# noveens/reviews4rec

Measured on AMD Instinct MI355X. Metric: train ratings/sec, higher is better.
Workload: dtype f32

## Files before the change

include/r4r.h:

```cpp
#ifndef R4R_H
#define R4R_H

#include <stddef.h>
#include <stdint.h>

#ifdef __cplusplus
extern "C" {
#endif

#define R4R_OK 0
#define R4R_ERR_ARG (-1)
#define R4R_ERR_LAUNCH (-2)
#define R4R_ERR_WORKSPACE (-3)

int r4r_version(void);
const char *r4r_last_error(void);

size_t r4r_textcnn_ws_bytes(int64_t N, int T, int E, int F, int64_t V);
int r4r_textcnn_fwd(const float *table, int64_t V, const int64_t *idx,
                    const float *conv_w, const float *conv_b,
                    float *pooled, int32_t *argmax,
                    void *ws, size_t ws_bytes,
                    int64_t N, int T, int E, int F, void *stream);

// ... 64 lines not shown
                       int64_t N, int R, int L, void *stream);

int r4r_mse_fwd_bwd(const float *out, const float *y, float *se, float *g_out,
                    int64_t N, float denom, void *stream);

int r4r_sqdist_mean_fwd(const float *a, const float *b, float *out, int64_t N, int L, void *stream);
int r4r_sqdist_mean_bwd(const float *a, const float *b, const float *g_out, float *g_a, float *g_b,
                        int64_t N, int L, void *stream);

int r4r_adam_chunk_elems(void);
int r4r_adam_multi(int ntensor, const uint64_t *p, const uint64_t *g, const uint64_t *m, const uint64_t *v,
                   const int64_t *numel, float lr, double beta1, double beta2, float eps,
                   float weight_decay, int64_t step, const int64_t *step_dev, void *stream);
int r4r_adam_gathered(float *p, const float *gathered, int world, float *g_sum, float *m, float *v,
                      int64_t numel, float lr, double beta1, double beta2, float eps,
                      float weight_decay, int64_t step, void *stream);
int r4r_adam_gathered_guarded(float *p, const float *gathered, int world, float *g_sum, float *m, float *v,
                              int64_t numel, float lr, double beta1, double beta2, float eps,
                              float weight_decay, int64_t step, const uint32_t *abort_word, void *stream);

int r4r_peer_segment_create(int64_t bytes, void **ptr, uint8_t *handle);
int r4r_peer_segment_open(const uint8_t *handle, void **ptr);
int r4r_peer_segment_close(void *ptr);
int r4r_peer_segment_destroy(void *ptr);
int r4r_peer_push(const float *src, int64_t numel, const uint64_t *peer_dst, const uint64_t *peer_flags,
                  uint32_t *arrive, int rank, int world, uint32_t epoch, const uint32_t *wait_flags,
                  uint32_t *timed_out, double timeout_s, void *stream);
int r4r_peer_wait(const uint32_t *flags, int world, uint32_t epoch, uint32_t *timed_out, double timeout_s, void *stream);


#define R4R_CONV_AUTO 0
#define R4R_CONV_DIRECT 1
#define R4R_CONV_PROJECT 2
int r4r_deepconn_nparam(void);
int r4r_deepconn_layout(int E, int L, int64_t *offsets, int64_t *sizes, int64_t *total);
size_t r4r_deepconn_ws_bytes(int64_t B, int T, int E, int L, int64_t V);
size_t r4r_deepconn_ws_mult_offset(int64_t B, int T, int E, int L, int64_t V);
size_t r4r_deepconn_ws_count_offset(int64_t B, int T, int E, int L, int64_t V, int tower, int buffer);
size_t r4r_deepconn_ws_partials_offset(int64_t B, int T, int E, int L, int64_t V, int tower, int which);
size_t r4r_deepconn_ws_plan_offset(int64_t B, int T, int E, int L, int64_t V, int tower, int buffer, int which);
size_t r4r_deepconn_ws_state_offset(int64_t B, int T, int E, int L, int64_t V, int tower, int buffer, int which);
int r4r_deepconn_step(const float *table, int64_t V, const int64_t *user_idx, const int64_t *item_idx,
                      const float *y, float *flat_p, float *flat_g,
                      float *pred, float *se, float *sse_accum,
                      void *ws, size_t ws_bytes,
                      int64_t B, int T, int E, int L,
                      float dropout_p, int training, uint64_t seed, uint64_t offset,
                      float inv_denom, int conv_algo, int token_buffer, int tokens_ready,
                      const int64_t *next_user_idx, const int64_t *next_item_idx,
                      float *flat_m, float *flat_v, float lr, double beta1, double beta2, float eps,
                      float weight_decay, int64_t adam_step, void *stream);
int r4r_deepconn_tail_fold(int on);
int r4r_deepconn_tail(int64_t B, int E, int L);
int r4r_deepconn_tokens(const int64_t *user_idx, const int64_t *item_idx, void *ws, size_t ws_bytes,
                        int64_t B, int T, int E, int L, int64_t V, int conv_algo, int token_buffer,
                        int discard, void *stream);

#define R4R_TIMING_TEXTCNN_FWD 0
#define R4R_TIMING_TEXTCNN_WGRAD 1
#define R4R_TIMING_ADAM 2
#define R4R_TIMING_PROJ_GEMM 3
#define R4R_TIMING_PROJ_GATHER 4
#define R4R_TIMING_SLOTS 8
int r4r_timing_enable(int slot_mask);
int r4r_timing_read(int slot, double *total_ms, int64_t *count, int reset);

size_t r4r_mf_ws_bytes(int64_t B, int D, int64_t n_users, int64_t n_items);
size_t r4r_mf_ws_persist_bytes(int64_t B, int D, int64_t n_users, int64_t n_items);
size_t r4r_mf_ws_mult_offset(int64_t B, int D, int64_t n_users, int64_t n_items);
size_t r4r_mf_ws_grad_offset(int64_t B, int D, int64_t n_users, int64_t n_items, int which);
int r4r_mf_step(const int64_t *uid, const int64_t *iid, const float *y,
                const uint64_t *p, const uint64_t *m, const uint64_t *v,
                int64_t n_users, int64_t n_items, int D,
                float *pred, float *se, float *sse_accum, void *ws, size_t ws_bytes, int64_t B,
                float dropout_p, int training, uint64_t seed, uint64_t offset, float inv_denom,
                int sweep_period, int64_t sweep_base, int sweep_all,
                float lr, double beta1, double beta2, float eps, float weight_decay, int64_t adam_step,
                void *stream);

int r4r_mf_rows_flush(const uint64_t *p, const uint64_t *m, const uint64_t *v,
                      int64_t n_users, int64_t n_items, int D, void *ws, size_t ws_bytes, int64_t B,
                      int sweep_period, int64_t sweep_base,
                      float lr, double beta1, double beta2, float eps, float weight_decay, int64_t adam_step,
                      void *stream);
size_t r4r_mf_ws_flag_offset(int64_t B, int D, int64_t n_users, int64_t n_items);

int r4r_sse_accumulate(const float *se, int64_t n, float *accum, void *stream);

size_t r4r_mf_dp_block_bytes(int64_t B_pad, int D);
int r4r_mf_grad(const int64_t *uid, const int64_t *iid, const float *y, const uint64_t *p,
                const uint64_t *m, const uint64_t *v,
                int64_t n_users, int64_t n_items, int D, float *pred, float *se, void *block, float *mult,
                int64_t B, int64_t B_pad, float dropout_p, int training, uint64_t seed, uint64_t offset,
                float inv_denom, void *ws, int sweep_period, int64_t sweep_base,
                float lr, double beta1, double beta2, float eps, float weight_decay, int64_t adam_step,
                void *stream);
int r4r_mf_apply(const void *blocks, int world, int64_t B_pad, const uint64_t *p, const uint64_t *m,
                 const uint64_t *v, int64_t n_users, int64_t n_items, int D, void *ws, size_t ws_bytes,
                 int sweep_period, int64_t sweep_base, int sweep_all,
                 const float *se, int64_t se_n, float *sse_accum,
                 float lr, double beta1, double beta2, float eps, float weight_decay, int64_t adam_step,
                 void *stream);
int r4r_mf_grad_push(const int64_t *uid, const int64_t *iid, const float *y, const uint64_t *p,
                     const uint64_t *m, const uint64_t *v,
                     int64_t n_users, int64_t n_items, int D, float *pred, float *se, float *mult,
                     int64_t B, int64_t B_pad, float dropout_p, int training, uint64_t seed, uint64_t offset,
// ... 380 lines not shown
```

reviews4rec_amd/csrc/engine.hip:

```cpp
#include <stdlib.h>

#include "trace_device.h"
#include "textcnn.h"
#include "wgrad_device.h"
#include "tokens_device.h"
#include "adam_device.h"

namespace r4r {

constexpr int F_CONV = 100;
constexpr int FM_K = 8;
constexpr int MAX_L = 128;

enum { P_UCW = 0, P_UCB, P_UFW, P_UFB, P_ICW, P_ICB, P_IFW, P_IFB, P_FMV, P_FMLW, P_FMLB, P_GB, P_COUNT };

struct Layout {
    int64_t off[P_COUNT], size[P_COUNT], total;
};

static Layout make_layout(int E, int L) {
    Layout lay;
    const int64_t sz[P_COUNT] = {(int64_t)F_CONV * 3 * E, F_CONV, (int64_t)L * F_CONV, L,
                                 (int64_t)F_CONV * 3 * E, F_CONV, (int64_t)L * F_CONV, L,
                                 (int64_t)2 * L * FM_K, 2 * L, 1, 1};
    int64_t o = 0;
    for (int i = 0; i < P_COUNT; ++i) {
        lay.off[i] = o;
        lay.size[i] = sz[i];
        o += (sz[i] + 31) & ~(int64_t)31;
    }
    lay.total = o;
    return lay;
}

struct HeadArgs {
    const float *pmax[2]; const int *parg[2];
    const float *fc_w[2]; const float *fc_b[2];
    const float *V, *lin_w, *lin_b, *gbias;
    const float *y;
    float *pooled[2]; int *argmax[2];
    float *g_pooled[2];
    float *mult;
    float *x, *s, *g, *gz;
    float *pred, *se;
    int64_t B;
    int L, tiles, training, want_grad;
    float p_drop, inv_denom;
    uint64_t seed, offset;
    PlanArgs plan;
    int *plan_spent[2];
    TokenArgs marks;
    int mark_wgs;
};


constexpr int HEAD_MAX_TILES = 8;

#define SEL2(arr, s) ((s) ? (arr)[1] : (arr)[0])
HEAD_TRACE_DEFINE(r4r_debug_dc_head_trace)
template <int ML>
__global__ __launch_bounds__(256) void deepconn_head_wg_kernel(HeadArgs a) {
    if ((int64_t)blockIdx.x >= a.B) {
        const int fb = (int)blockIdx.x - (int)a.B, flag_wgs = (2 * a.plan.units + 3) / 4;
        if (fb < flag_wgs) {
            segment_flags_wave(a.plan, fb * 4 + (int)(threadIdx.x >> 6));
        } else {
            const HeadArgs &A = kernel_args<HeadArgs>();
            token_mark_block(A.marks, fb - flag_wgs, A.mark_wgs, 256);
        }
        return;
    }
    HEAD_STAMP(0)
    constexpr int N2 = 2 * ML, PARTS = 256 / N2;
    __shared__ float sw[2][ML][F_CONV + 1];
    __shared__ float sfb[N2], slw[N2], sz[N2];
    __shared__ float sV[N2][FM_K];
    __shared__ float sp[2][F_CONV + 4];
    __shared__ float red[N2][PARTS + 1];
    const int tid = threadIdx.x, lane = tid & 63, w = tid >> 6;
    const int64_t b = blockIdx.x;
    const int L = a.L, n = 2 * L;
    const float lin_b0 = a.lin_b[0], gbias0 = a.gbias[0], yb = a.y ? a.y[b] : 0.f;

    constexpr int FQ = F_CONV / 4;
    typedef float hq4 __attribute__((ext_vector_type(4)));
    constexpr int WREGS = (2 * ML * FQ + 255) / 256;
    hq4 wreg[WREGS];
    const int wtot = 2 * L * FQ;
#pragma unroll
    for (int k = 0; k < WREGS; ++k) {
        const int i = min(tid + 256 * k, wtot - 1);
        const int t = i >= L * FQ;
        wreg[k] = *reinterpret_cast<const hq4 *>(SEL2(a.fc_w, t) + 4 * (i - t * L * FQ));
    }
    const int tn = min(tid, n - 1);
    const float fbreg = SEL2(a.fc_b, tn >= L)[tn - (tn >= L ? L : 0)];
    const float lwreg = a.lin_w[tn];
    constexpr int VREGS = (N2 * FM_K + 255) / 256;
    float vreg[VREGS];
#pragma unroll
    for (int k = 0; k < VREGS; ++k) vreg[k] = a.V[min(tid + 256 * k, n * FM_K - 1)];
    if (b == 0 && tid < 2 && SEL2(a.plan_spent, tid)) SEL2(a.plan_spent, tid)[0] = 0;

    {
        const int t = w >> 1, f = lane + 64 * (w & 1), fc = min(f, F_CONV - 1);
        float best = -INFINITY;
        int bp = -1;
        if (a.tiles <= HEAD_MAX_TILES) {
            float v[HEAD_MAX_TILES];
            int pp[HEAD_MAX_TILES];
#pragma unroll
            for (int k = 0; k < HEAD_MAX_TILES; ++k) {
                const size_t o = ((size_t)b * a.tiles + min(k, a.tiles - 1)) * NP + fc;
                v[k] = SEL2(a.pmax, t)[o];
                pp[k] = SEL2(a.parg, t)[o];
            }
#pragma unroll
            for (int k = 0; k < HEAD_MAX_TILES; ++k)
                if (v[k] > best) { best = v[k]; bp = pp[k]; }
        } else {
            for (int k0 = 0; k0 < a.tiles; k0 += HEAD_MAX_TILES) {
                float v[HEAD_MAX_TILES];
                int pp[HEAD_MAX_TILES];
#pragma unroll
                for (int k = 0; k < HEAD_MAX_TILES; ++k) {
                    const bool in = k0 + k < a.tiles;
                    const size_t o = ((size_t)b * a.tiles + (in ? k0 + k : 0)) * NP + fc;
                    v[k] = in ? SEL2(a.pmax, t)[o] : -INFINITY;
                    pp[k] = SEL2(a.parg, t)[o];
                }
#pragma unroll
                for (int k = 0; k < HEAD_MAX_TILES; ++k)
                    if (v[k] > best) { best = v[k]; bp = pp[k]; }
            }
        }
        if (!(best > 0.f)) { best = 0.f; bp = -1; }
        if (f < F_CONV) {
            sp[t][f] = best;
            SEL2(a.pooled, t)[b * F_CONV + f] = best;
            SEL2(a.argmax, t)[b * F_CONV + f] = bp;
        }
    }
    HEAD_STAMP(1)
#pragma unroll
    for (int k = 0; k < WREGS; ++k) {
        const int i = tid + 256 * k;
        if (i < wtot) {
            const int t = i >= L * FQ, r = i - t * L * FQ, l = r / FQ, f0 = 4 * (r - l * FQ);
#pragma unroll
            for (int c = 0; c < 4; ++c) sw[t][l][f0 + c] = wreg[k][c];
        }
    }
    if (tid < n) { sfb[tid] = fbreg; slw[tid] = lwreg; }
#pragma unroll
    for (int k = 0; k < VREGS; ++k) {
        const int i = tid + 256 * k;
        if (i < n * FM_K) sV[i / FM_K][i % FM_K] = vreg[k];
    }
    __syncthreads();
    HEAD_STAMP(2)

    {
        const int o = tid / PARTS, part = tid - o * PARTS;
        if (o < n) {
            const int t = o / L, l = o - t * L;
            float acc = 0.f;
            for (int f = part; f < F_CONV; f += PARTS) acc = fmaf(sp[t][f], sw[t][l][f], acc);
            red[o][part] = acc;
        }
    }
    __syncthreads();
    const bool has_y = a.y != nullptr, want = has_y && a.want_grad;
    if (w == 0) {
        constexpr int NI = (N2 + 63) / 64;
        float xi[NI], mult[NI], lw[NI], gacc[NI];
#pragma unroll
        for (int u = 0; u < NI; ++u) {
            const int i = lane + 64 * u;
            xi[u] = 0.f; mult[u] = 1.f; gacc[u] = 0.f;
            lw[u] = (i < n) ? slw[i] : 0.f;
            if (i < n) {
                float acc = 0.f;
#pragma unroll
                for (int q = 0; q < PARTS; ++q) acc += red[i][q];
                xi[u] = acc + sfb[i];
            }
            if (a.training && a.p_drop > 0.f && i < n) {
                const uint32_t r = philox_first_word(a.offset + (uint64_t)(b * n + i), a.seed);
                const float uu = (float)(r >> 8) * (1.0f / 16777216.0f);
                mult[u] = (uu >= a.p_drop) ? 1.f / (1.f - a.p_drop) : 0.f;
            }
            xi[u] *= mult[u];
        }
        float inter = 0.f;
        float sk_keep[FM_K];
#pragma unroll
        for (int k = 0; k < FM_K; ++k) {
            float pv = 0.f, pv2 = 0.f, vv[NI];
#pragma unroll
            for (int u = 0; u < NI; ++u) {
                const int i = lane + 64 * u;
                vv[u] = (i < n) ? sV[i][k] : 0.f;
                pv += xi[u] * vv[u];
                pv2 += xi[u] * xi[u] * vv[u] * vv[u];
            }
            const float sk = wave_sum(pv);
            const float s2 = wave_sum(pv2);
            inter += sk * sk - s2;
#pragma unroll
            for (int u = 0; u < NI; ++u) gacc[u] += sk * vv[u] - xi[u] * vv[u] * vv[u];
            sk_keep[k] = sk;
        }
        float pl = 0.f;
#pragma unroll
        for (int u = 0; u < NI; ++u) pl += xi[u] * lw[u];
        const float lin = wave_sum(pl);
        const float pred = (0.5f * inter + lin + lin_b0) + gbias0;
        if (lane == 0) a.pred[b] = pred;
        if (has_y) {
            const float d = pred - yb;
            if (lane == 0) a.se[b] = d * d;
            if (want) {
                const float g = 2.f * d * a.inv_denom;
#pragma unroll
                for (int u = 0; u < NI; ++u) {
                    const int i = lane + 64 * u;
                    const float gx = g * (gacc[u] + lw[u]);
                    const float gz = gx * mult[u];
                    if (i < n) {
                        sz[i] = gz;
                        a.x[b * n + i] = xi[u];
                        a.gz[b * n + i] = gz;
                        a.mult[b * n + i] = mult[u];
                    }
                }
                if (lane < FM_K) {
                    float sv = 0.f;
#pragma unroll
                    for (int k = 0; k < FM_K; ++k) if (lane == k) sv = sk_keep[k];
                    a.s[b * FM_K + lane] = sv;
                }
                if (lane == 0) a.g[b] = g;
            }
        }
    }
    if (!want) return;
    __syncthreads();
    HEAD_STAMP(3)
    if (tid < 2 * F_CONV) {
        const int t = tid >= F_CONV, f = tid - t * F_CONV;
        float acc = 0.f;
        for (int l = 0; l < L; ++l) acc = fmaf(sz[t * L + l], sw[t][l][f], acc);
        SEL2(a.g_pooled, t)[b * F_CONV + f] = acc;
    }
    HEAD_STAMP(4)
}

struct HeadGradArgs {
    const float *pooled[2];
    const float *x, *s, *g, *gz;
    const float *V;
    const float *se;
    float *g_fc_w[2], *g_fc_b[2], *g_V, *g_lin_w, *g_lin_b, *g_gb;
    float *sse_accum;
    int64_t B;
    int L;
};

constexpr int HG_ROWS = 16, HG_COLS = 16;
template <bool STEP = false>
__device__ __forceinline__ void head_grad_block(const HeadGradArgs &a, int blk, const FlatAdam *opt = nullptr) {
    __shared__ float red[HG_ROWS][HG_COLS];
    const int ox = threadIdx.x & (HG_COLS - 1), rg = threadIdx.x / HG_COLS;
    const int L = a.L, n = 2 * L;
    const int n_fcw = L * F_CONV;
    const int seg[9] = {n_fcw, L, n_fcw, L, n * FM_K, n, 1, 1, 1};
    int o = blk * HG_COLS + ox;
    int which = -1, local = 0, acc_o = o;
#pragma unroll
    for (int k = 0; k < 9; ++k) {
        if (which < 0) {
            if (acc_o < seg[k]) { which = k; local = acc_o; }
            else acc_o -= seg[k];
        }
    }
    float P = 0.f, M = 0.f, V = 0.f;
    int po = 0;
    bool stepping = false;
    if constexpr (STEP) {
        if (opt->on && rg == 0 && which >= 0 && which < 8) {
            const float *dst = which == 0 ? a.g_fc_w[0] + local : (which == 1 ? a.g_fc_b[0] + local : (which == 2 ? a.g_fc_w[1] + local :
                  (which == 3 ? a.g_fc_b[1] + local : (which == 4 ? a.g_V + local : (which == 5 ? a.g_lin_w + local :
                  (which == 6 ? a.g_lin_b : a.g_gb))))));
            po = (int)(dst - opt->g);
            stepping = true;
        }
    }
    float s = 0.f;
    if (which >= 0) {
// ... 50 lines not shown
        }
        if constexpr (STEP) {
            if (stepping) {
                adam_elem(P, t, M, V, opt->s);
                opt->p[po] = P; opt->m[po] = M; opt->v[po] = V;
            }
        }
    }
}

BWD_TRACE_DEFINE(r4r_debug_dc_bwd_trace)
struct DcBackwardArgs {
    WgradArgs w;
    HeadGradArgs h;
    int hg_blocks;
    TokenArgs nx;
    PlanArgs plan;
};
__global__ __launch_bounds__(WG_THREADS, 8) void deepconn_backward_kernel(DcBackwardArgs) {
    const DcBackwardArgs &A = kernel_args<DcBackwardArgs>();
    const WgradArgs &w = A.w;
    const HeadGradArgs &h = A.h;
    const TokenArgs &nx = A.nx;
    const PlanArgs &plan = A.plan;
    const int hg_blocks = A.hg_blocks;
    BWD_STAMP(0, wall_clock64())
    BWD_STAMP(2, (unsigned long long)blockIdx.z + 1)
    if (blockIdx.z == 1 || blockIdx.z == 2) {
        wgrad_block(w, blockIdx.x, blockIdx.y, blockIdx.z - 1);
    } else if (blockIdx.z == 0) {
        for (int blk = blockIdx.y * gridDim.x + blockIdx.x; blk < hg_blocks; blk += gridDim.x * gridDim.y) {
            head_grad_block(h, blk);
            __syncthreads();
        }
    } else {
        const int np = plan.units > 0 ? 2 : 0, blk = blockIdx.y * gridDim.x + blockIdx.x;
        if (blk < np) segment_plan_block<WG_THREADS>(plan, blk);
        else token_mark_block(nx, blk - np, gridDim.x * gridDim.y - np, WG_THREADS);
    }
#ifdef R4R_TRACE
    __syncthreads();
#endif
    BWD_STAMP(1, wall_clock64())
}

struct DcFoldArgs {
    WgradArgs w;
    FlatAdam opt;
    HeadGradArgs h;
    int hg_blocks;
    TokenArgs nx;
    PlanArgs plan;
    int comp_blocks;
};
static_assert(WG_THREADS % 64 == 0, "the 256-thread roles of the fold launch are whole waves: the others end before any barrier");
template <bool BIGV>
__global__ __launch_bounds__(WG_ROW_MAX_THREADS, 8) void deepconn_backward_fold_kernel(DcFoldArgs) {
    const DcFoldArgs &A = kernel_args<DcFoldArgs>();
    BWD_STAMP(0, wall_clock64())
    BWD_STAMP(2, (unsigned long long)blockIdx.z + 1)
    if (blockIdx.z == 1 || blockIdx.z == 2) {
        wgrad_row_block(A.w, A.opt, blockIdx.x, blockIdx.y, blockIdx.z - 1);
    } else {
        if (threadIdx.x >= WG_THREADS) return;
        const int blk0 = blockIdx.y * gridDim.x + blockIdx.x, nblk = gridDim.x * gridDim.y;
        if (blockIdx.z == 0) {
            for (int blk = blk0; blk < A.hg_blocks; blk += nblk) {
                head_grad_block<true>(A.h, blk, &A.opt);
                __syncthreads();
            }
        } else {
            const int np = A.plan.units > 0 ? 2 : 0, comp_blocks = A.comp_blocks;
            const int blk = ((int)blockIdx.z - 3) * nblk + blk0;
            if (blk < np) {
                segment_plan_block<WG_THREADS>(A.plan, blk);
            } else if (blk - np < 2 * comp_blocks) {
                const int t = (blk - np) >= comp_blocks;
                const TokenTower &tw = t ? A.nx.t[1] : A.nx.t[0];
                if constexpr (BIGV) token_compact_block<WG_THREADS / 64, COMPACT_BIG_G>(tw, A.nx.V, blk - np - t * comp_blocks);
                else token_compact_block<WG_THREADS / 64, 1>(tw, A.nx.V, blk - np - t * comp_blocks);
            }
        }
    }
#ifdef R4R_TRACE
    __syncthreads();
#endif
    BWD_STAMP(1, wall_clock64())
}

constexpr int RED_THREADS = 256;
struct FusedAdam {
    float *p, *m, *v;
    const float *g;
    int64_t lo[2], hi[2];
    AdamScalars s;
    int on;
};
__global__ __launch_bounds__(RED_THREADS) void deepconn_reduce_kernel(WgradArgs w, int red_blocks, int comp_blocks,
                                                                      TokenArgs nx, FusedAdam opt) {
    const int bx = blockIdx.x;
    if (bx < red_blocks) {
        const WgradTower &tw = w.t[blockIdx.y];
        const int nw = w.F * 3 * w.E;
        const int i = bx * RED_THREADS + threadIdx.x;
        const float *gp0 = i < nw ? tw.d_w + i : (i < nw + w.F ? tw.d_b + (i - nw) : nullptr);
        const int64_t o = gp0 ? gp0 - opt.g : 0;
        float P = 0.f, M = 0.f, V = 0.f;
        if (opt.on && gp0) { P = opt.p[o]; M = opt.m[o]; V = opt.v[o]; }
        float *dst;
        const float g = wgrad_reduce_elem(w, blockIdx.y, i, dst);
        if (opt.on && dst) {
            adam_elem(P, g, M, V, opt.s);
            opt.p[o] = P; opt.m[o] = M; opt.v[o] = V;
        }
    } else if (bx < red_blocks + comp_blocks) {
        token_compact_auto<RED_THREADS / 64>(nx.t[blockIdx.y], nx.V, bx - red_blocks);
    } else {
        const int64_t o = opt.lo[blockIdx.y] + (int64_t)(bx - red_blocks - comp_blocks) * RED_THREADS + threadIdx.x;
        if (o < opt.hi[blockIdx.y]) {
            float P = opt.p[o], M = opt.m[o], V = opt.v[o];
            adam_elem(P, opt.g[o], M, V, opt.s);
            opt.p[o] = P; opt.m[o] = M; opt.v[o] = V;
        }
    }
}

__global__ void sse_only_kernel(const float *__restrict__ se, float *__restrict__ accum, int64_t B) {
    __shared__ float red[256];
    float s = 0.f;
    for (int64_t i = threadIdx.x; i < B; i += 256) s += se[i];
    red[threadIdx.x] = s;
    __syncthreads();
    for (int off = 128; off > 0; off >>= 1) {
        if ((int)threadIdx.x < off) red[threadIdx.x] += red[threadIdx.x + off];
        __syncthreads();
    }
    if (threadIdx.x == 0) accum[0] += red[0];
}

struct StepWs {
    float *wp[2], *pmax[2]; int *parg[2];
    int *flags[2][2], *slot[2][2], *list[2][2], *count[2][2]; float *ptab[2];
    int *live[2][2], *perm[2][2], *plan_ready[2][2];
    float *pooled[2]; int *argmax[2]; float *g_pooled[2];
    float *mult, *x, *s, *g, *gz;
    float *part_w[2], *part_b[2];
    size_t bytes;
};

static StepWs carve(void *ws, int64_t B, int T, int E, int L, int64_t V) {
    StepWs w;
    char *p = static_cast<char *>(ws);
    auto take = [&](size_t nbytes) { char *r = p; p += align256(nbytes); return r; };
    const size_t tiles128 = (size_t)(T + 2 + 127) / 128;
    const int ns = textcnn_wgrad_splits(B);
    for (int t = 0; t < 2; ++t) {
        w.wp[t] = reinterpret_cast<float *>(take(textcnn_wp_floats(E) * 4));
        w.pmax[t] = reinterpret_cast<float *>(take((size_t)B * tiles128 * NP * 4));
        w.parg[t] = reinterpret_cast<int *>(take((size_t)B * tiles128 * NP * 4));
        w.pooled[t] = reinterpret_cast<float *>(take((size_t)B * F_CONV * 4));
        w.argmax[t] = reinterpret_cast<int *>(take((size_t)B * F_CONV * 4));
        w.g_pooled[t] = reinterpret_cast<float *>(take((size_t)B * F_CONV * 4));
        w.part_w[t] = reinterpret_cast<float *>(take((size_t)ns * F_CONV * 3 * E * 4));
        w.part_b[t] = reinterpret_cast<float *>(take((size_t)ns * F_CONV * 4));
        for (int bf = 0; bf < 2; ++bf) {
            w.flags[bf][t] = reinterpret_cast<int *>(take((size_t)(V + 4) * 4));
            w.slot[bf][t] = reinterpret_cast<int *>(take((size_t)(V + 4) * 4));
            w.list[bf][t] = reinterpret_cast<int *>(take((size_t)proj_row_capacity(B, T, V) * 4));
            w.count[bf][t] = reinterpret_cast<int *>(take(256));
        }
        w.ptab[t] = reinterpret_cast<float *>(take(proj_ptab_floats(B, T, V) * 4));
    }
    w.mult = reinterpret_cast<float *>(take((size_t)B * 2 * L * 4));
    w.x = reinterpret_cast<float *>(take((size_t)B * 2 * L * 4));
    w.gz = reinterpret_cast<float *>(take((size_t)B * 2 * L * 4));
    w.s = reinterpret_cast<float *>(take((size_t)B * FM_K * 4));
    w.g = reinterpret_cast<float *>(take((size_t)B * 4));
    for (int t = 0; t < 2; ++t)
        for (int bf = 0; bf < 2; ++bf) {
            w.live[bf][t] = reinterpret_cast<int *>(take((size_t)PLAN_MAX_UNITS * 4));
            w.perm[bf][t] = reinterpret_cast<int *>(take((size_t)PLAN_MAX_UNITS * 4));
            w.plan_ready[bf][t] = reinterpret_cast<int *>(take(256));
        }
    w.bytes = (size_t)(p - static_cast<char *>(ws));
    return w;
}

}

using namespace r4r;

extern "C" int r4r_deepconn_nparam(void) { return P_COUNT; }

extern "C" int r4r_deepconn_layout(int E, int L, int64_t *offsets, int64_t *sizes, int64_t *total) {
    R4R_REQUIRE(E > 0 && L > 0 && L <= MAX_L && offsets && sizes && total, "deepconn_layout: bad arguments");
    const Layout lay = make_layout(E, L);
    for (int i = 0; i < P_COUNT; ++i) { offsets[i] = lay.off[i]; sizes[i] = lay.size[i]; }
    *total = lay.total;
    return R4R_OK;
}

extern "C" size_t r4r_deepconn_ws_bytes(int64_t B, int T, int E, int L, int64_t V) {
    if (B < 0 || T <= 0 || E <= 0 || L <= 0 || V <= 0) return 0;
    return carve(nullptr, B, T, E, L, V).bytes;
}

extern "C" size_t r4r_deepconn_ws_mult_offset(int64_t B, int T, int E, int L, int64_t V) {
    char base[1];
    const StepWs w = carve(base, B, T, E, L, V);
    return (size_t)(reinterpret_cast<char *>(w.mult) - base);
}

extern "C" size_t r4r_deepconn_ws_count_offset(int64_t B, int T, int E, int L, int64_t V, int tower, int buffer) {
    char base[1];
    const StepWs w = carve(base, B, T, E, L, V);
    return (size_t)(reinterpret_cast<char *>(w.count[buffer & 1][tower & 1]) - base);
}

extern "C" size_t r4r_deepconn_ws_partials_offset(int64_t B, int T, int E, int L, int64_t V, int tower, int which) {
    char base[1];
    const StepWs w = carve(base, B, T, E, L, V);
    const void *at = which ? static_cast<const void *>(w.parg[tower & 1]) : w.pmax[tower & 1];
    return (size_t)(static_cast<const char *>(at) - base);
}
extern "C" size_t r4r_deepconn_ws_plan_offset(int64_t B, int T, int E, int L, int64_t V, int tower, int buffer, int which) {
    char base[1];
    const StepWs w = carve(base, B, T, E, L, V);
    const int t = tower & 1, bf = buffer & 1;
    const void *at[3] = {w.perm[bf][t], w.plan_ready[bf][t], w.live[bf][t]};
    return (which < 0 || which > 2) ? 0 : (size_t)(static_cast<const char *>(at[which]) - base);
}

extern "C" size_t r4r_deepconn_ws_state_offset(int64_t B, int T, int E, int L, int64_t V, int tower, int buffer, int which) {
    char base[1];
    const StepWs w = carve(base, B, T, E, L, V);
    const int t = tower & 1, bf = buffer & 1;
    const void *at[4] = {w.flags[bf][t], w.slot[bf][t], w.list[bf][t], w.argmax[t]};
    return (which < 0 || which > 3) ? 0 : (size_t)(static_cast<const char *>(at[which]) - base);
}

static bool plan_applies(int64_t B, int T) {
    const int tiles = proj_tiles(T);
    return proj_gather_plan() && (tiles & 1) == 0 && B * tiles <= PLAN_MAX_UNITS;
}

static int g_tail_fold = -1;
static int tail_fold_switch() {
    if (g_tail_fold < 0) {
        const char *e = getenv("R4R_TAIL");
        g_tail_fold = (e && e[0] == 'o') ? 0 : 1;
    }
    return g_tail_fold;
}
static bool tail_folds(int64_t B, int E, int L) {
    if (!tail_fold_switch() || B < 1 || E <= 0 || E % 4 != 0 || L > 64) return false;
    const int ns = textcnn_wgrad_splits(B);
    return wgrad_row_applies(B, E, ns, (int)cdiv(B, ns));
}
extern "C" int r4r_deepconn_tail_fold(int on) {
    const int before = tail_fold_switch();
    g_tail_fold = on ? 1 : 0;
    return before;
}
extern "C" int r4r_deepconn_tail(int64_t B, int E, int L) { return tail_folds(B, E, L) ? 1 : 0; }

extern "C" int r4r_deepconn_tokens(const int64_t *user_idx, const int64_t *item_idx, void *ws, size_t ws_bytes,
                                   int64_t B, int T, int E, int L, int64_t V, int conv_algo, int token_buffer,
                                   int discard, void *stream) {
    R4R_REQUIRE(user_idx && item_idx && ws, "deepconn_tokens: null pointer");
    R4R_REQUIRE(token_buffer == 0 || token_buffer == 1, "deepconn_tokens: token_buffer must be 0 or 1");
    if (ws_bytes < r4r_deepconn_ws_bytes(B, T, E, L, V)) {
        set_error("deepconn_tokens: workspace %zu < %zu bytes", ws_bytes, r4r_deepconn_ws_bytes(B, T, E, L, V));
        return R4R_ERR_WORKSPACE;
    }
    if (B == 0 || textcnn_pick_algo(conv_algo, B, T, E, F_CONV) != R4R_CONV_PROJECT) return R4R_OK;
    const StepWs w = carve(ws, B, T, E, L, V);
    if (discard) {
        for (int t = 0; t < 2; ++t) {
            (void)hipMemsetAsync(w.count[token_buffer][t], 0, sizeof(int), as_stream(stream));
            (void)hipMemsetAsync(w.plan_ready[token_buffer][t], 0, sizeof(int), as_stream(stream));
        }
        return check_launch("deepconn_tokens(discard)");
    }
    ProjTower pt[2];
    const int64_t *idx[2] = {user_idx, item_idx};
    for (int t = 0; t < 2; ++t) {
        pt[t] = ProjTower{};
        pt[t].idx = idx[t];
        pt[t].flags = w.flags[token_buffer][t]; pt[t].slot = w.slot[token_buffer][t];
        pt[t].list = w.list[token_buffer][t]; pt[t].count = w.count[token_buffer][t];
    }
    return textcnn_proj_tokens_launch(V, pt, 2, B, T, false, as_stream(stream));
}

extern "C" int r4r_deepconn_step(const float *table, int64_t V, const int64_t *user_idx, const int64_t *item_idx,
                                 const float *y, float *flat_p, float *flat_g,
                                 float *pred, float *se, float *sse_accum,
                                 void *ws, size_t ws_bytes,
                                 int64_t B, int T, int E, int L,
                                 float dropout_p, int training, uint64_t seed, uint64_t offset,
                                 float inv_denom, int conv_algo, int token_buffer, int tokens_ready,
                                 const int64_t *next_user_idx, const int64_t *next_item_idx,
                                 float *flat_m, float *flat_v, float lr, double beta1, double beta2, float eps,
                                 float weight_decay, int64_t adam_step,
                                 void *stream) {
    R4R_REQUIRE(table && user_idx && item_idx && flat_p && pred && ws, "deepconn_step: null pointer");
    R4R_REQUIRE(!flat_m == !flat_v, "deepconn_step: flat_m and flat_v go together");
    R4R_REQUIRE(!flat_m || (flat_g && adam_step >= 1), "deepconn_step: the fused optimiser needs gradients and "
                                                       "adam_step >= 1");
    R4R_REQUIRE(!next_user_idx == !next_item_idx, "deepconn_step: next_user_idx and next_item_idx go together");
    R4R_REQUIRE(!next_user_idx || flat_g, "deepconn_step: the next batch's tokens ride on the backward launches "
                                          "(training steps only)");
    R4R_REQUIRE(V > 0 && B >= 0 && T > 0, "deepconn_step: bad sizes");
    R4R_REQUIRE(E > 0 && E % 4 == 0, "deepconn_step: word_embed_size %d must be a positive multiple of 4", E);
    R4R_REQUIRE(L > 0 && L <= MAX_L, "deepconn_step: latent_size %d outside 1..%d", L, MAX_L);
    R4R_REQUIRE(!flat_g || (y && se), "deepconn_step: gradients need ratings y and the se buffer");
    R4R_REQUIRE(!y || se, "deepconn_step: se buffer required when y is given");
// ... 21 lines not shown
    if (algo == R4R_CONV_PROJECT) {
        ProjTower pt[2];
        for (int t = 0; t < 2; ++t) {
            pt[t].idx = idx[t];
            pt[t].conv_w = P[t ? P_ICW : P_UCW];
            pt[t].conv_b = P[t ? P_ICB : P_UCB];
            pt[t].flags = w.flags[token_buffer][t]; pt[t].slot = w.slot[token_buffer][t];
            pt[t].list = w.list[token_buffer][t]; pt[t].count = w.count[token_buffer][t];
            pt[t].ptab = w.ptab[t]; pt[t].pmax = w.pmax[t]; pt[t].parg = w.parg[t]; pt[t].wimg = w.wp[t];
            if (tokens_ready && plan_applies(B, T)) {
                pt[t].perm = w.perm[token_buffer][t]; pt[t].plan_ready = w.plan_ready[token_buffer][t];
            }
        }
        if (!tokens_ready)
            if (int rc = textcnn_proj_tokens_launch(V, pt, 2, B, T, false, st)) return rc;
        if (int rc = textcnn_proj_compute_launch(table, V, pt, 2, B, T, E, F_CONV, st)) return rc;
        tiles = proj_tiles(T);
    } else {
        FwdTower ft[2];
        for (int t = 0; t < 2; ++t) {
            ft[t].idx = idx[t];
            ft[t].conv_w = P[t ? P_ICW : P_UCW];
            ft[t].conv_b = P[t ? P_ICB : P_UCB];
            ft[t].wp = w.wp[t]; ft[t].pmax = w.pmax[t]; ft[t].parg = w.parg[t];
        }
        if (int rc = textcnn_fwd_launch(table, ft, 2, B, T, E, F_CONV, st)) return rc;
        tiles = textcnn_tiles(T);
    }

    HeadArgs h;
    for (int t = 0; t < 2; ++t) {
        h.pmax[t] = w.pmax[t]; h.parg[t] = w.parg[t];
        h.fc_w[t] = P[t ? P_IFW : P_UFW]; h.fc_b[t] = P[t ? P_IFB : P_UFB];
        h.pooled[t] = w.pooled[t]; h.argmax[t] = w.argmax[t]; h.g_pooled[t] = w.g_pooled[t];
    }
    h.V = P[P_FMV]; h.lin_w = P[P_FMLW]; h.lin_b = P[P_FMLB]; h.gbias = P[P_GB];
    h.y = y; h.mult = w.mult; h.x = w.x; h.s = w.s; h.g = w.g; h.gz = w.gz;
    h.pred = pred; h.se = se;
    h.B = B; h.L = L; h.tiles = tiles; h.training = training; h.want_grad = flat_g != nullptr;
    h.p_drop = dropout_p; h.inv_denom = inv_denom; h.seed = seed; h.offset = offset;
    const bool planning = next_user_idx && flat_g && algo == R4R_CONV_PROJECT && plan_applies(B, T);
    PlanArgs plan{};
    if (planning) {
        const int ob = token_buffer ^ 1;
        plan.idx[0] = next_user_idx; plan.idx[1] = next_item_idx;
        for (int t = 0; t < 2; ++t) {
            plan.live[t] = w.live[ob][t]; plan.perm[t] = w.perm[ob][t]; plan.plan_ready[t] = w.plan_ready[ob][t];
        }
        plan.T = T; plan.tiles = proj_tiles(T); plan.units = (int)(B * plan.tiles);
    }
    h.plan = plan;
    for (int t = 0; t < 2; ++t) h.plan_spent[t] = algo == R4R_CONV_PROJECT ? w.plan_ready[token_buffer][t] : nullptr;
    const bool fold = flat_g && tail_folds(B, E, L);
    const bool prefetch = next_user_idx && algo == R4R_CONV_PROJECT;
    TokenArgs nx{};
    if (prefetch) {
        ProjTower nt[2];
        const int64_t *nidx[2] = {next_user_idx, next_item_idx};
        const int ob = token_buffer ^ 1;
        for (int t = 0; t < 2; ++t) {
            nt[t] = ProjTower{};
            nt[t].idx = nidx[t];
            nt[t].flags = w.flags[ob][t]; nt[t].slot = w.slot[ob][t];
            nt[t].list = w.list[ob][t]; nt[t].count = w.count[ob][t];
        }
        nx = make_token_args(V, nt, 2, B, T);
    }
    h.marks = nx;
    const int64_t mark_want = cdiv(B * (int64_t)T, 256);
    h.mark_wgs = (fold && prefetch) ? (int)(mark_want < 1024 ? mark_want : 1024) : 0;
    const unsigned head_wgs = (unsigned)B + (unsigned)cdiv(2 * (int64_t)plan.units, 4) + (unsigned)h.mark_wgs;
    if (L <= 16) deepconn_head_wg_kernel<16><<<head_wgs, 256, 0, st>>>(h);
    else if (L <= 32) deepconn_head_wg_kernel<32><<<head_wgs, 256, 0, st>>>(h);
    else if (L <= 64) deepconn_head_wg_kernel<64><<<head_wgs, 256, 0, st>>>(h);
    else deepconn_head_wg_kernel<128><<<head_wgs, 256, 0, st>>>(h);

    if (!flat_g) {
        if (y && sse_accum) sse_only_kernel<<<1, 256, 0, st>>>(se, sse_accum, B);
        return check_launch("deepconn_step(forward)");
    }

    HeadGradArgs hg;
    for (int t = 0; t < 2; ++t) {
        hg.pooled[t] = w.pooled[t];
        hg.g_fc_w[t] = G[t ? P_IFW : P_UFW]; hg.g_fc_b[t] = G[t ? P_IFB : P_UFB];
    }
    hg.x = w.x; hg.s = w.s; hg.g = w.g; hg.gz = w.gz; hg.V = P[P_FMV]; hg.se = se;
    hg.g_V = G[P_FMV]; hg.g_lin_w = G[P_FMLW]; hg.g_lin_b = G[P_FMLB]; hg.g_gb = G[P_GB];
    hg.sse_accum = sse_accum; hg.B = B; hg.L = L;
    const int nout = 2 * (L * F_CONV + L) + 2 * L * FM_K + 2 * L + 3;
    const int hg_blocks = (nout + HG_COLS - 1) / HG_COLS;

    WgradTower wt[2];
    WgradArgs wa;
    for (int t = 0; t < 2; ++t) {
        wt[t].idx = idx[t]; wt[t].g_pooled = w.g_pooled[t]; wt[t].argmax = w.argmax[t];
        wt[t].part_w = w.part_w[t]; wt[t].part_b = w.part_b[t];
        wt[t].d_w = G[t ? P_ICW : P_UCW]; wt[t].d_b = G[t ? P_ICB : P_UCB];
    }
    for (int k = 0; k < MAX_TOWERS; ++k) wa.t[k] = wt[k < 2 ? k : 0];
    wa.table = table; wa.N = B; wa.T = T; wa.E = E; wa.F = F_CONV;
    wa.table_bytes = (int64_t)V * E * 4;
    wa.nsplit = textcnn_wgrad_splits(B);
    wa.per_split = (int)cdiv(B, wa.nsplit);
    const int comp_blocks = prefetch ? (int)cdiv((V + 3) / 4, RED_THREADS * compact_groups(V)) : 0;
    if (fold) {
        FlatAdam fo{};
        if (flat_m) {
            fo.on = 1;
            fo.p = flat_p; fo.m = flat_m; fo.v = flat_v; fo.g = flat_g;
            fo.s = adam_make_scalars(lr, beta1, beta2, eps, weight_decay, adam_step, nullptr);
        }
        const int side = prefetch ? (planning ? 2 : 0) + 2 * comp_blocks : 0;
        const unsigned nz = 3 + (unsigned)cdiv(side, F_CONV * 3);
        {
            ScopedTiming tm(R4R_TIMING_TEXTCNN_WGRAD, st);
            const DcFoldArgs fa{wa, fo, hg, hg_blocks, nx, plan, comp_blocks};
            const dim3 grid(F_CONV, 3, nz);
            const int nthr = wgrad_row_threads(E, wa.nsplit);
            if (V > COMPACT_BIG_V) deepconn_backward_fold_kernel<true><<<grid, nthr, 0, st>>>(fa);
            else deepconn_backward_fold_kernel<false><<<grid, nthr, 0, st>>>(fa);
        }
        return check_launch("deepconn_step");
    }
    {
        ScopedTiming tm(R4R_TIMING_TEXTCNN_WGRAD, st);
        deepconn_backward_kernel<<<dim3(F_CONV, wa.nsplit, prefetch ? 4 : 3), WG_THREADS, 0, st>>>(DcBackwardArgs{wa, hg, hg_blocks, nx, plan});
    }
    const int red_blocks = (F_CONV * 3 * E + F_CONV + RED_THREADS - 1) / RED_THREADS;
    FusedAdam opt{};
    int opt_blocks = 0;
    if (flat_m) {
        opt.on = 1;
        opt.p = flat_p; opt.m = flat_m; opt.v = flat_v; opt.g = flat_g;
        opt.lo[0] = lay.off[P_UFW]; opt.hi[0] = lay.off[P_ICW];
        opt.lo[1] = lay.off[P_IFW]; opt.hi[1] = lay.total;
        opt.s = adam_make_scalars(lr, beta1, beta2, eps, weight_decay, adam_step, nullptr);
        const int64_t longest = opt.hi[0] - opt.lo[0] > opt.hi[1] - opt.lo[1] ? opt.hi[0] - opt.lo[0] : opt.hi[1] - opt.lo[1];
        opt_blocks = (int)cdiv(longest, RED_THREADS);
    }
    deepconn_reduce_kernel<<<dim3(red_blocks + comp_blocks + opt_blocks, 2), RED_THREADS, 0, st>>>(
        wa, red_blocks, comp_blocks, nx, opt);
    return check_launch("deepconn_step");
}

extern "C" int r4r_sse_accumulate(const float *se, int64_t n, float *accum, void *stream) {
    R4R_REQUIRE(accum && (se || n == 0) && n >= 0, "sse_accumulate: bad arguments");
    if (n == 0) return R4R_OK;
    sse_only_kernel<<<1, 256, 0, as_stream(stream)>>>(se, accum, n);
    return check_launch("sse_accumulate");
}
```

reviews4rec_amd/csrc/wgrad_device.h:

```cpp
#pragma once
#include "adam_device.h"
#include "textcnn.h"

namespace r4r {

typedef float wg_f32x4 __attribute__((ext_vector_type(4)));

constexpr int WG_THREADS = 256;

struct WgradArgs {
    WgradTower t[MAX_TOWERS];
    const float *table;
    int64_t N;
    int T, E, F, per_split, nsplit;
    int64_t table_bytes = 0;
};

constexpr int WG_CHUNK = 16;
constexpr int WG_FLIGHT = 8;

template <bool FIRST>
__device__ __forceinline__ void wgrad_block_pass(const WgradArgs &a, int f, int s, int tower, int v0,
                                                 long (&s_off)[WG_CHUNK][3], float (&s_g)[WG_CHUNK]) {
    const WgradTower &tw = a.t[tower];
// ... 156 lines not shown
                    v[d] = *reinterpret_cast<const wg_f32x4 *>(table + (off < 0 ? 0 : off) + ve);
                }
#pragma unroll
                for (int d = 0; d < WG_CHUNK; ++d) {
                    const wg_f32x4 sum = acc + p_g[wave][r0 + d] * v[d];
                    acc = p_off[wave][r0 + d][vj] >= 0 ? sum : acc;
                }
            }
        }
        if (live && lane == 0)
            for (int d = 0; d < nd; ++d) sb += p_g[wave][d];
    }
    if (live && lane < nvec) *reinterpret_cast<wg_f32x4 *>(tw.part_w + ((size_t)s * F + f) * 3 * E + lane * 4) = acc;
    if (live && lane == 0) tw.part_b[(size_t)s * F + f] = sb;
}

constexpr int WG_MAX_SPLITS = 16;

__device__ __forceinline__ float wgrad_reduce_elem(const WgradArgs &a, int tower, int i, float *&dst) {
    const WgradTower &tw = a.t[tower];
    const int nw = a.F * 3 * a.E;
    const float *src;
    size_t stride;
    if (i < nw) { src = tw.part_w + i; stride = (size_t)nw; dst = tw.d_w + i; }
    else if (i < nw + a.F) { src = tw.part_b + (i - nw); stride = (size_t)a.F; dst = tw.d_b + (i - nw); }
    else { dst = nullptr; return 0.f; }
    float v[WG_MAX_SPLITS];
#pragma unroll
    for (int k = 0; k < WG_MAX_SPLITS; ++k) v[k] = src[(size_t)(k < a.nsplit ? k : 0) * stride];
    float s = 0.f;
#pragma unroll
    for (int k = 0; k < WG_MAX_SPLITS; ++k)
        if (k < a.nsplit) s += v[k];
    *dst = s;
    return s;
}

__device__ __forceinline__ void wgrad_reduce_block(const WgradArgs &a, int tower, int blk) {
    float *dst;
    (void)wgrad_reduce_elem(a, tower, blk * (int)blockDim.x + (int)threadIdx.x, dst);
}

constexpr int WG_ROW_MAX_THREADS = 1024;
constexpr int WG_ROW_MAX_DOCS = WG_MAX_SPLITS * WG_CHUNK;
constexpr unsigned WG_ROW_NONE = 0xffffffffu;
inline bool wgrad_row_applies(int64_t N, int E, int nsplit, int per_split) {
    return N >= 1 && N <= WG_ROW_MAX_DOCS && per_split <= WG_CHUNK && nsplit <= WG_MAX_SPLITS && E % 4 == 0 &&
           (int64_t)nsplit * (E / 4) <= WG_ROW_MAX_THREADS;
}
inline int wgrad_row_threads(int E, int nsplit) {
    const int t = (nsplit * (E / 4) + 63) & ~63;
    return t < WG_THREADS ? WG_THREADS : t;
}
__device__ __forceinline__ void wgrad_row_block(const WgradArgs &a, const FlatAdam &opt, int f, int tap, int tower) {
    __shared__ long r_off[WG_ROW_MAX_DOCS];
    __shared__ unsigned r_bo[WG_ROW_MAX_DOCS];
    __shared__ float r_g[WG_ROW_MAX_DOCS];
    __shared__ __attribute__((aligned(16))) float r_part[4 * WG_ROW_MAX_THREADS];
    __shared__ float r_sb[WG_MAX_SPLITS];
    const WgradTower &tw = a.t[tower];
    const float *__restrict__ table = a.table;
    const int T = a.T, E = a.E, F = a.F, e4 = E / 4, nsplit = a.nsplit;
    const int N = (int)a.N;
    const int tid = threadIdx.x;
    const int s = tid / e4, c = tid - s * e4, ve = 4 * c;
    const bool worker = s < nsplit;
    const int tot = E + (tap == 0 ? 1 : 0);
    float *const row_w = tw.d_w + ((size_t)f * 3 + tap) * E;
    float *const dst0 = tid < E ? row_w + tid : tw.d_b + f;
    float P = 0.f, M = 0.f, V = 0.f;
    if (opt.on && tid < tot) {
        const int o = (int)(dst0 - opt.g);
        P = opt.p[o]; M = opt.m[o]; V = opt.v[o];
    }
    if (tid < N) {
        const int p = tw.argmax[(int64_t)tid * F + f];
        const float gv = tw.g_pooled[(int64_t)tid * F + f];
        const int t = p - 2 + tap;
        long off = -1;
        if (p >= 0 && t >= 0 && t < T) off = (long)tw.idx[(int64_t)tid * T + t] * E;
        r_off[tid] = off;
        r_bo[tid] = off >= 0 ? (unsigned)(off * 4) : WG_ROW_NONE;
        r_g[tid] = (p >= 0) ? gv : 0.f;
    }
    __syncthreads();
    const int n0 = worker ? s * a.per_split : 0;
    const int nd = worker ? max(0, min(N, n0 + a.per_split) - n0) : 0;
    wg_f32x4 acc = {0.f, 0.f, 0.f, 0.f};
    const bool buf_ok = a.table_bytes > 0 && a.table_bytes < (1ll << 32);
    const __amdgpu_buffer_rsrc_t rsrc = __builtin_amdgcn_make_buffer_rsrc(const_cast<float *>(table), 0, buf_ok ? (int)(unsigned)a.table_bytes : 0, 0x00020000);
    if (worker && nd > 0) {
        if (buf_ok) {
#pragma unroll
            for (int d0 = 0; d0 < WG_CHUNK; d0 += WG_FLIGHT) {
                wg_f32x4 row[WG_FLIGHT];
                bool on[WG_FLIGHT];
#pragma unroll
                for (int u = 0; u < WG_FLIGHT; ++u) {
                    const int d = d0 + u;
                    const unsigned rv = r_bo[n0 + d];
                    const unsigned ro = d < nd ? rv : WG_ROW_NONE;
                    on[u] = ro != WG_ROW_NONE;
                    const unsigned bo = on[u] ? ro + (unsigned)(ve * 4) : 0xfffffff0u;
                    row[u] = __builtin_bit_cast(wg_f32x4, __builtin_amdgcn_raw_buffer_load_b128(rsrc, (int)bo, 0, 0));
                }
#pragma unroll
                for (int u = 0; u < WG_FLIGHT; ++u) {
                    const wg_f32x4 sum = acc + r_g[n0 + d0 + u] * row[u];
                    acc = on[u] ? sum : acc;
                }
                __builtin_amdgcn_sched_barrier(0);
            }
        } else {
#pragma unroll 4
            for (int d = 0; d < nd; ++d) {
                const long off = r_off[n0 + d];
                if (off >= 0) acc += r_g[n0 + d] * *reinterpret_cast<const wg_f32x4 *>(table + off + ve);
            }
        }
    }
    r_part[4 * tid] = acc.x; r_part[4 * tid + 1] = acc.y; r_part[4 * tid + 2] = acc.z; r_part[4 * tid + 3] = acc.w;
    if (tap == 0 && tid < nsplit) {
        const int b0 = tid * a.per_split, bn = max(0, min(N, b0 + a.per_split) - b0);
        float sb = 0.f;
        for (int d = 0; d < bn; ++d) sb += r_g[b0 + d];
        r_sb[tid] = sb;
    }
    __syncthreads();
// ... 19 lines not shown
```

Baseline: 1.446 million.

## Resolve argmax token ids in head kernel and hand them to wgrad

The DeepCoNN head kernel now looks up the token id under each tap of every filter's argmax window while it does its FC/FM work. It writes these ids to a new per-tower workspace buffer. The fused backward wgrad row block then reads the ready ids instead of the dependent argmax→idx load chain, taking that latency off the backward critical path. The trade is extra loads and stores in the head kernel plus more workspace. The path is on by default when the tail fold is active, and for L>64 it launches the ML=64 variant, which looks inconsistent with the non-ATOK path.

```diff
diff --git a/include/r4r.h b/include/r4r.h
--- a/include/r4r.h
+++ b/include/r4r.h
@@ -140,6 +140,8 @@
                       float weight_decay, int64_t adam_step, void *stream);
 int r4r_deepconn_tail_fold(int on);
 int r4r_deepconn_tail(int64_t B, int E, int L);
+int r4r_deepconn_atok(int on);
+size_t r4r_deepconn_ws_atok_offset(int64_t B, int T, int E, int L, int64_t V, int tower);
 int r4r_deepconn_tokens(const int64_t *user_idx, const int64_t *item_idx, void *ws, size_t ws_bytes,
                         int64_t B, int T, int E, int L, int64_t V, int conv_algo, int token_buffer,
                         int discard, void *stream);
diff --git a/reviews4rec_amd/csrc/engine.hip b/reviews4rec_amd/csrc/engine.hip
--- a/reviews4rec_amd/csrc/engine.hip
+++ b/reviews4rec_amd/csrc/engine.hip
@@ -51,6 +51,9 @@
     int *plan_spent[2];
     TokenArgs marks;
     int mark_wgs;
+    const int64_t *idx[2];
+    int *atok[2];
+    int T;
 };
 
 
@@ -58,7 +61,7 @@
 
 #define SEL2(arr, s) ((s) ? (arr)[1] : (arr)[0])
 HEAD_TRACE_DEFINE(r4r_debug_dc_head_trace)
-template <int ML>
+template <int ML, bool ATOK = false>
 __global__ __launch_bounds__(256) void deepconn_head_wg_kernel(HeadArgs a) {
     if ((int64_t)blockIdx.x >= a.B) {
         const int fb = (int)blockIdx.x - (int)a.B, flag_wgs = (2 * a.plan.units + 3) / 4;
@@ -77,6 +80,7 @@
     __shared__ float sV[N2][FM_K];
     __shared__ float sp[2][F_CONV + 4];
     __shared__ float red[N2][PARTS + 1];
+    __shared__ int sarg[2][F_CONV + 4];
     const int tid = threadIdx.x, lane = tid & 63, w = tid >> 6;
     const int64_t b = blockIdx.x;
     const int L = a.L, n = 2 * L;
@@ -140,6 +144,8 @@
             SEL2(a.pooled, t)[b * F_CONV + f] = best;
             SEL2(a.argmax, t)[b * F_CONV + f] = bp;
         }
+        if constexpr (ATOK)
+            if (f < F_CONV) sarg[t][f] = bp;
     }
     HEAD_STAMP(1)
 #pragma unroll
@@ -159,6 +165,18 @@
     }
     __syncthreads();
     HEAD_STAMP(2)
+    constexpr int ATOK_ITEMS = 2 * F_CONV * 3, ATOK_PER = (ATOK_ITEMS + 191) / 192;
+    [[maybe_unused]] int atk[ATOK_PER];
+    if constexpr (ATOK) {
+        if (w > 0) {
+#pragma unroll
+            for (int k = 0; k < ATOK_PER; ++k) {
+                const int i = min(tid - 64 + 192 * k, ATOK_ITEMS - 1), tf = i / 3, j = i - tf * 3, t = tf >= F_CONV;
+                const int tp = sarg[t][tf - t * F_CONV] - 2 + j;
+                atk[k] = reinterpret_cast<const int *>(SEL2(a.idx, t) + b * a.T)[2 * min(max(tp, 0), a.T - 1)];
+            }
+        }
+    }
 
     {
         const int o = tid / PARTS, part = tid - o * PARTS;
@@ -245,6 +263,19 @@
         }
     }
     if (!want) return;
+    if constexpr (ATOK) {
+        if (w > 0) {
+            static_assert(ATOK_PER == 4, "the four ids named below");
+            asm volatile("" : "+v"(atk[0]), "+v"(atk[1]), "+v"(atk[2]), "+v"(atk[3]));
+#pragma unroll
+            for (int k = 0; k < ATOK_PER; ++k) {
+                const int i = tid - 64 + 192 * k, tf = min(i, ATOK_ITEMS - 1) / 3, j = i - tf * 3, t = tf >= F_CONV;
+                const int bp = sarg[t][tf - t * F_CONV], tp = bp - 2 + j;
+                if (i < ATOK_ITEMS)
+                    SEL2(a.atok, t)[b * (F_CONV * 3) + (i - t * F_CONV * 3)] = (bp >= 0 && tp >= 0 && tp < a.T) ? atk[k] : -1;
+            }
+        }
+    }
     __syncthreads();
     HEAD_STAMP(3)
     if (tid < 2 * F_CONV) {
@@ -401,6 +432,7 @@
     TokenArgs nx;
     PlanArgs plan;
     int comp_blocks;
+    const int *atok[2];
 };
 static_assert(WG_THREADS % 64 == 0, "the 256-thread roles of the fold launch are whole waves: the others end before any barrier");
 template <bool BIGV>
@@ -409,7 +441,7 @@
     BWD_STAMP(0, wall_clock64())
     BWD_STAMP(2, (unsigned long long)blockIdx.z + 1)
     if (blockIdx.z == 1 || blockIdx.z == 2) {
-        wgrad_row_block(A.w, A.opt, blockIdx.x, blockIdx.y, blockIdx.z - 1);
+        wgrad_row_block(A.w, A.opt, blockIdx.x, blockIdx.y, blockIdx.z - 1, blockIdx.z == 1 ? A.atok[0] : A.atok[1]);
     } else {
         if (threadIdx.x >= WG_THREADS) return;
         const int blk0 = blockIdx.y * gridDim.x + blockIdx.x, nblk = gridDim.x * gridDim.y;
@@ -494,6 +526,7 @@
     float *pooled[2]; int *argmax[2]; float *g_pooled[2];
     float *mult, *x, *s, *g, *gz;
     float *part_w[2], *part_b[2];
+    int *atok[2];
     size_t bytes;
 };
 
@@ -531,6 +564,7 @@
             w.perm[bf][t] = reinterpret_cast<int *>(take((size_t)PLAN_MAX_UNITS * 4));
             w.plan_ready[bf][t] = reinterpret_cast<int *>(take(256));
         }
+    for (int t = 0; t < 2; ++t) w.atok[t] = reinterpret_cast<int *>(take((size_t)B * F_CONV * 3 * 4));
     w.bytes = (size_t)(p - static_cast<char *>(ws));
     return w;
 }
@@ -588,6 +622,12 @@
     return (which < 0 || which > 3) ? 0 : (size_t)(static_cast<const char *>(at[which]) - base);
 }
 
+extern "C" size_t r4r_deepconn_ws_atok_offset(int64_t B, int T, int E, int L, int64_t V, int tower) {
+    char base[1];
+    const StepWs w = carve(base, B, T, E, L, V);
+    return (size_t)(reinterpret_cast<char *>(w.atok[tower & 1]) - base);
+}
+
 static bool plan_applies(int64_t B, int T) {
     const int tiles = proj_tiles(T);
     return proj_gather_plan() && (tiles & 1) == 0 && B * tiles <= PLAN_MAX_UNITS;
@@ -612,6 +652,20 @@
     return before;
 }
 extern "C" int r4r_deepconn_tail(int64_t B, int E, int L) { return tail_folds(B, E, L) ? 1 : 0; }
+
+static int g_atok = -1;
+static int atok_switch() {
+    if (g_atok < 0) {
+        const char *e = getenv("R4R_ATOK");
+        g_atok = (e && e[0] == '0') ? 0 : 1;
+    }
+    return g_atok;
+}
+extern "C" int r4r_deepconn_atok(int on) {
+    const int before = atok_switch();
+    g_atok = on ? 1 : 0;
+    return before;
+}
 
 extern "C" int r4r_deepconn_tokens(const int64_t *user_idx, const int64_t *item_idx, void *ws, size_t ws_bytes,
                                    int64_t B, int T, int E, int L, int64_t V, int conv_algo, int token_buffer,
@@ -739,6 +793,9 @@
     h.plan = plan;
     for (int t = 0; t < 2; ++t) h.plan_spent[t] = algo == R4R_CONV_PROJECT ? w.plan_ready[token_buffer][t] : nullptr;
     const bool fold = flat_g && tail_folds(B, E, L);
+    const bool hand_tokens = fold && atok_switch();
+    for (int t = 0; t < 2; ++t) { h.idx[t] = idx[t]; h.atok[t] = hand_tokens ? w.atok[t] : nullptr; }
+    h.T = T;
     const bool prefetch = next_user_idx && algo == R4R_CONV_PROJECT;
     TokenArgs nx{};
     if (prefetch) {
@@ -757,7 +814,11 @@
     const int64_t mark_want = cdiv(B * (int64_t)T, 256);
     h.mark_wgs = (fold && prefetch) ? (int)(mark_want < 1024 ? mark_want : 1024) : 0;
     const unsigned head_wgs = (unsigned)B + (unsigned)cdiv(2 * (int64_t)plan.units, 4) + (unsigned)h.mark_wgs;
-    if (L <= 16) deepconn_head_wg_kernel<16><<<head_wgs, 256, 0, st>>>(h);
+    if (hand_tokens) {
+        if (L <= 16) deepconn_head_wg_kernel<16, true><<<head_wgs, 256, 0, st>>>(h);
+        else if (L <= 32) deepconn_head_wg_kernel<32, true><<<head_wgs, 256, 0, st>>>(h);
+        else deepconn_head_wg_kernel<64, true><<<head_wgs, 256, 0, st>>>(h);
+    } else if (L <= 16) deepconn_head_wg_kernel<16><<<head_wgs, 256, 0, st>>>(h);
     else if (L <= 32) deepconn_head_wg_kernel<32><<<head_wgs, 256, 0, st>>>(h);
     else if (L <= 64) deepconn_head_wg_kernel<64><<<head_wgs, 256, 0, st>>>(h);
     else deepconn_head_wg_kernel<128><<<head_wgs, 256, 0, st>>>(h);
@@ -802,7 +863,8 @@
         const unsigned nz = 3 + (unsigned)cdiv(side, F_CONV * 3);
         {
             ScopedTiming tm(R4R_TIMING_TEXTCNN_WGRAD, st);
-            const DcFoldArgs fa{wa, fo, hg, hg_blocks, nx, plan, comp_blocks};
+            const DcFoldArgs fa{wa, fo, hg, hg_blocks, nx, plan, comp_blocks,
+                                {hand_tokens ? w.atok[0] : nullptr, hand_tokens ? w.atok[1] : nullptr}};
             const dim3 grid(F_CONV, 3, nz);
             const int nthr = wgrad_row_threads(E, wa.nsplit);
             if (V > COMPACT_BIG_V) deepconn_backward_fold_kernel<true><<<grid, nthr, 0, st>>>(fa);
diff --git a/reviews4rec_amd/csrc/wgrad_device.h b/reviews4rec_amd/csrc/wgrad_device.h
--- a/reviews4rec_amd/csrc/wgrad_device.h
+++ b/reviews4rec_amd/csrc/wgrad_device.h
@@ -232,7 +232,8 @@
     const int t = (nsplit * (E / 4) + 63) & ~63;
     return t < WG_THREADS ? WG_THREADS : t;
 }
-__device__ __forceinline__ void wgrad_row_block(const WgradArgs &a, const FlatAdam &opt, int f, int tap, int tower) {
+__device__ __forceinline__ void wgrad_row_block(const WgradArgs &a, const FlatAdam &opt, int f, int tap, int tower,
+                                                const int *__restrict__ atok = nullptr) {
     __shared__ long r_off[WG_ROW_MAX_DOCS];
     __shared__ unsigned r_bo[WG_ROW_MAX_DOCS];
     __shared__ float r_g[WG_ROW_MAX_DOCS];
@@ -253,7 +254,18 @@
         const int o = (int)(dst0 - opt.g);
         P = opt.p[o]; M = opt.m[o]; V = opt.v[o];
     }
-    if (tid < N) {
+    if (atok) {
+        if (tid < N) {
+            const int *at = atok + ((int64_t)tid * F + f) * 3;
+            const int a0 = at[0], a1 = at[1], a2 = at[2];
+            const float gv = tw.g_pooled[(int64_t)tid * F + f];
+            const int tok = tap == 0 ? a0 : (tap == 1 ? a1 : a2);
+            const long off = tok >= 0 ? (long)tok * E : -1;
+            r_off[tid] = off;
+            r_bo[tid] = off >= 0 ? (unsigned)(off * 4) : WG_ROW_NONE;
+            r_g[tid] = ((a0 & a1 & a2) >= 0) ? gv : 0.f;
+        }
+    } else if (tid < N) {
         const int p = tw.argmax[(int64_t)tid * F + f];
         const float gv = tw.g_pooled[(int64_t)tid * F + f];
         const int t = p - 2 + tap;
```

Measured after the change: 1.448 million (median of 4 runs). No clear change (+0.1%).
